# aponte411/minGPT-distributed

Measured on AMD Instinct MI355X. Metric: tokens/sec (whole node), GPT-2 124M seq1024 bf16, higher is better.
Workload: dtype bf16; 1 GPU; model=gpt2, global_batch=128, seq_len=1024, parallelism=dp1, micro_batch_per_gpu=128, hip_graph=False

## Files before the change

### csrc/bindings.cpp

```cpp
#include <torch/extension.h>
#include <ATen/hip/impl/HIPGuardImplMasqueradingAsCUDA.h>
#include <ATen/hip/impl/HIPStreamMasqueradingAsCUDA.h>

#include "comm.h"
#include "kernels.h"

namespace {

using mg::bf16_t;

hipStream_t cur_stream() { return c10::hip::getCurrentHIPStreamMasqueradingAsCUDA().stream(); }
using DevGuard = c10::hip::HIPGuardMasqueradingAsCUDA;

#define CHECK_DEV(t) TORCH_CHECK((t).is_cuda(), #t " must be a GPU tensor")
#define CHECK_CONTIG(t) TORCH_CHECK((t).is_contiguous(), #t " must be contiguous")
#define CHECK_BF16(t) \
  CHECK_DEV(t);       \
  TORCH_CHECK((t).scalar_type() == at::kBFloat16, #t " must be bf16")
#define CHECK_F32(t) \
  CHECK_DEV(t);      \
  TORCH_CHECK((t).scalar_type() == at::kFloat, #t " must be fp32")
#define CHECK_I64(t) \
  CHECK_DEV(t);      \
  TORCH_CHECK((t).scalar_type() == at::kLong, #t " must be int64")
// ... 858 lines not shown
  m.def("xent_scale_", &xent_scale_);
  m.def("set_graph_state", &set_graph_state, py::arg("seed_ofs") = py::none(), py::arg("opt_hp") = py::none());
  m.def("grad_sumsq", &grad_sumsq);
  m.def("grad_sumsq_chunks", &grad_sumsq_chunks);
  m.def("adamw_step", &adamw_step, py::arg("chunk_start"), py::arg("chunk_len"), py::arg("chunk_wd"),
        py::arg("moment_start"), py::arg("master"), py::arg("param"), py::arg("grad"), py::arg("m"),
        py::arg("v"), py::arg("norm"), py::arg("lr"), py::arg("b1"), py::arg("b2"), py::arg("eps"),
        py::arg("step"), py::arg("grad_scale"), py::arg("clip"), py::arg("table_end"),
        py::arg("moment_end"), py::arg("zero_grad") = py::none());
  m.def("f32_to_bf16", &f32_to_bf16);
  m.def("comm_proxy", &comm_proxy);
  m.def("bias_act", &bias_act);
  m.def("bias_dropout_residual", &bias_dropout_residual);
  m.def("gelu_bwd", &gelu_bwd);
  m.def("dropout_bwd", &dropout_bwd);
  m.def("transpose", &transpose);
  m.def("bias_grad", &bias_grad);
  m.def("dropout_bias_grad", &dropout_bias_grad);
  m.def("gemm", &gemm, py::arg("a"), py::arg("b"), py::arg("c"), py::arg("layout"), py::arg("epi"),
        py::arg("bias"), py::arg("aux"), py::arg("resid"), py::arg("p"), py::arg("seed"), py::arg("M"),
        py::arg("N"), py::arg("dbias") = py::none());
  m.def("gemm_set_variant", &mg::gemm_set_variant);
  m.def("gemm_get_variant", &mg::gemm_get_variant);
  m.def("gemm_pick", &mg::gemm_pick, py::arg("M"), py::arg("N"), py::arg("K"), py::arg("layout"));
  m.def("attention_set_bwd_mode", &mg::attention_set_bwd_mode);
  m.def("attention_set_bwd64", &mg::attention_set_bwd64);
#ifdef MG_BWD64_STAMPS
  m.def("attention_bwd64_stamps", []() {
    auto t = at::empty({64 * 4 * 8 * 8 + 64 * 4 * 16}, at::kLong);
    mg::attention_bwd64_stamps(reinterpret_cast<unsigned long long*>(t.data_ptr<int64_t>()));
    return t;
  });
#endif
  m.def("attention_fwd", &attention_fwd);
  m.def("attention_bwd", &attention_bwd, py::arg("qkv"), py::arg("out"), py::arg("dout"), py::arg("lse"),
        py::arg("mask"), py::arg("B"), py::arg("T"), py::arg("H"), py::arg("p"), py::arg("seed"),
        py::arg("dbias") = py::none());
  m.def("gemv", &gemv, py::arg("x"), py::arg("W"), py::arg("epi"), py::arg("bias") = py::none(),
        py::arg("resid") = py::none(), py::arg("ldy") = 0, py::arg("lnw") = py::none(),
        py::arg("lnb") = py::none(), py::arg("eps") = 1e-5, py::arg("am_part") = py::none(),
        py::arg("am_pos") = py::none());
  m.def("gemv_argmax_groups", [](int64_t N, int64_t B) { return (int64_t)mg::gemv_grid((int)N, (int)B); },
        py::arg("N"), py::arg("B"));
  m.def("gemv_supported", &mg::gemv_supported);
  m.def("attention_decode", &attention_decode, py::arg("qkv_new"), py::arg("cache"), py::arg("H"),
        py::arg("pos"), py::arg("pos_dev") = py::none(), py::arg("part") = py::none(),
// ... 22 lines not shown
```

### csrc/include/kernels.h

```cpp
#pragma once
#include <hip/hip_runtime.h>
#include <stddef.h>
#include <stdint.h>

namespace mg {
typedef uint16_t bf16_t;

void layernorm_fwd(const bf16_t* x, const bf16_t* w, const bf16_t* b, bf16_t* y, float* mean,
                   float* rstd, int M, int D, float eps, hipStream_t stream);
void layernorm_bwd(const bf16_t* dy, const bf16_t* x, const bf16_t* w, const float* mean,
                   const float* rstd, const bf16_t* dres, bf16_t* dx, float* dw, float* db,
                   float* workspace, int M, int D, hipStream_t stream, bf16_t* dz = nullptr,
                   float* dzb = nullptr, float p = 0.f, uint64_t seed = 0);
size_t layernorm_bwd_workspace(int M, int D, bool drop);

void embedding_fwd(const int64_t* idx, const bf16_t* wte, const bf16_t* wpe, bf16_t* out, int M,
                   int T, int D, int V, float p, uint64_t seed, hipStream_t stream,
                   const int* pos_dev = nullptr,
                   const unsigned long long* am_part = nullptr,
                   int am_groups = 0,
                   int64_t* tok = nullptr,
                   int64_t* seq = nullptr,
                   long seq_ld = 0,
                   int pos_stride = 0,
// ... 56 lines not shown
void beam_merge(int B, int W, int V, const int* cand_tok, const float* cand_c, float* score, int* fin, int* len,
                int64_t* tok, int* parent, int* hist_parent, int* hist_tok, float* hist_score, long hist_ld, int* pos,
                const int* ctl, hipStream_t stream);
void beam_reorder(bf16_t* kv, int L, long layer_stride, int B, int W, int Tmax, int D, const int* parent,
                  const int* pos, int* ctl, hipStream_t stream);

void bias_act_fwd(const bf16_t* x, const bf16_t* b, bf16_t* pre, bf16_t* y, long M, int N, int act,
                  hipStream_t stream);
void bias_dropout_residual(const bf16_t* x, const bf16_t* b, const bf16_t* r, bf16_t* y, long M,
                           int N, float p, uint64_t seed, hipStream_t stream);
void gelu_bwd(const bf16_t* dy, const bf16_t* pre, bf16_t* dx, long n, hipStream_t stream);
void dropout_bwd(const bf16_t* dy, bf16_t* dx, long M, int N, float p, uint64_t seed, hipStream_t stream);
void transpose(const bf16_t* src, bf16_t* dst, int R, int C, int ldd, hipStream_t stream);
void bias_grad(const bf16_t* dy, float* db, long M, int N, hipStream_t stream, long ld = 0);
void dropout_bias_grad(const bf16_t* dy, bf16_t* dx, float* db, long M, int N, float p, uint64_t seed,
                       hipStream_t stream);

void gemm(int layout, int epi, const bf16_t* A, const bf16_t* B, void* C, long lda, long ldb,
          long ldc, int M, int N, int K, int a_ext, int b_ext, int ka, int kb, const bf16_t* bias,
          bf16_t* aux, const bf16_t* resid, float p, uint64_t seed, hipStream_t stream,
          size_t a_bytes, size_t b_bytes,
          float* dbias = nullptr);
void gemm_set_variant(int v);
void gemm_set_debug_buffer(unsigned long long* p);
int gemm_get_variant();
int gemm_pick(int M, int N, int K, int layout);

size_t attention_dropout_mask_words(int B, int T, int H);
int attention_dropout_threshold(float p);
float attention_dropout_scale(int thr);
void attention_fwd(const bf16_t* qkv, bf16_t* out, float* lse, uint32_t* dmask, int B, int T, int H,
                   int hd, float p, uint64_t seed, hipStream_t stream);
size_t attention_bwd_workspace_floats(int B, int T, int H, int hd);
void attention_set_bwd_mode(int mode);
void attention_set_bwd64(int on);
#ifdef MG_BWD64_STAMPS
void attention_bwd64_stamps(unsigned long long* host);
#endif
void attention_bwd(const bf16_t* qkv, const bf16_t* out, const bf16_t* dout, const float* lse,
                   const uint32_t* dmask, float* delta, float* dq, bf16_t* dqkv, int B, int T, int H,
                   int hd, float p, uint64_t seed, hipStream_t stream, float* dbias = nullptr);

size_t attention_decode_part_floats(int B, int H, int hd);
void attention_decode(const bf16_t* qkv_new, bf16_t* cache, bf16_t* out, int B, int H, int hd,
                      long Tmax, int pos, hipStream_t stream, float* part, unsigned* counters,
                      const int* pos_dev = nullptr, int pos_stride = 0);
// ... 3 lines not shown
```

### csrc/kernels/gemm.hip

```cpp
#include "common.h"
#include "kernels.h"
#include <type_traits>


using namespace mg;

namespace {

typedef __bf16 bf16x8 __attribute__((ext_vector_type(8)));
typedef __attribute__((address_space(3))) s16x4 lds_s16x4;
typedef __attribute__((address_space(3))) void lds_void;

constexpr int BK = 64;
#ifndef MG_GROUP_M
#define MG_GROUP_M 8
#endif
constexpr int GROUP_M = MG_GROUP_M;
constexpr uint32_t kOOB = 0xFFFFFFF0u;

template <int BM_, int BN_, int NWM_, int NWN_, int STAGES_ = 2>
struct Cfg {
  static constexpr int BM = BM_, BN = BN_, NWM = NWM_, NWN = NWN_, STAGES = STAGES_;
  static constexpr int NW = NWM * NWN, NT = NW * 64;
  static constexpr int WTM = BM / NWM, WTN = BN / NWN;
// ... 58 lines not shown
    ptr = reinterpret_cast<const char*>(p);
    total = tot;
    ld = ld_;
    kbeg = kbeg_;
    step = KC ? BK * 2 : (uint32_t)(BK * ld * 2);
    klim = min(kvalid, kend) - kbeg;
    tail_t = klim / BK;
    swid = __builtin_amdgcn_readfirstlane(wid);
#pragma unroll
    for (int i = 0; i < PER; ++i) {
      const int j = wid * PER + i;
      if constexpr (KC) {
        const int row = 8 * j + (lane >> 3), ch = (lane & 7) ^ (row & 7);
        voff[i] = (uint32_t)(((long)row * ld + ch * 8) * 2);
      } else {
        const int half = j >> 4, jj = j & 15;
        const int row = 4 * jj + (lane >> 4), ch = (lane & 15) ^ swz_mn(row);
        const int gc = r0 + half * 128 + ch * 8;
        voff[i] = gc < ext ? (uint32_t)(((long)row * ld + gc) * 2) : kOOB;
      }
    }
    retarget(r0);
  }
  MG_DEVICE void retarget(int r0) {
    const uint64_t o = KC ? (uint64_t)((long)r0 * ld + kbeg) * 2 : (uint64_t)kbeg * ld * 2;
    base = ptr + o;
    const uint64_t rest = total > o ? total - o : 0u;
    bytes = rest < 0xFFFFFF00u ? (uint32_t)rest : 0xFFFFFF00u;
  }
  MG_DEVICE __amdgpu_buffer_rsrc_t rsrc(int t) const { return tile_rsrc(base, bytes, step, t); }
  MG_DEVICE void piece(char* lds, __amdgpu_buffer_rsrc_t rs, int t, int i, bool check = true) const {
    const int j = swid * PER + i;
    uint32_t off = voff[i];
    if (check && t >= tail_t) {
      const int lane = threadIdx.x & 63;
      const int kpos = KC ? ((lane & 7) ^ ((lane >> 3) & 7)) * 8 : 4 * (j & 15) + (lane >> 4);
      off = kpos < klim - t * BK ? off : kOOB;
    }
    char* dst = KC ? lds + j * 1024 : lds + (j >> 4) * HS + (j & 15) * 1024;
    __builtin_amdgcn_raw_ptr_buffer_load_lds(rs, (lds_void*)dst, 16, off, 0, 0, 0);
  }
  MG_DEVICE void stage(char* lds, int t) const {
    const __amdgpu_buffer_rsrc_t rs = tile_rsrc(base, bytes, step, t);
#pragma unroll
    for (int i = 0; i < PER; ++i) piece(lds, rs, t, i);
  }
};

MG_DEVICE uint32_t lds_addr(const void* p) {
  return (uint32_t)(uintptr_t)(const __attribute__((address_space(3))) void*)p;
}
// ... 43 lines not shown
MG_DEVICE uint4 load8(const bf16_t* p, int valid) {
  if (valid >= 8) return *reinterpret_cast<const uint4*>(p);
  uint16_t t[8];
#pragma unroll
  for (int e = 0; e < 8; ++e) t[e] = e < valid ? p[e] : (uint16_t)0;
  return make_uint4(t[0] | (uint32_t)t[1] << 16, t[2] | (uint32_t)t[3] << 16, t[4] | (uint32_t)t[5] << 16,
                    t[6] | (uint32_t)t[7] << 16);
}

MG_DEVICE void store8(bf16_t* p, uint4 v, int valid) {
  if (valid >= 8) {
    *reinterpret_cast<uint4*>(p) = v;
    return;
  }
  const uint32_t w[4] = {v.x, v.y, v.z, v.w};
#pragma unroll
  for (int e = 0; e < 8; ++e)
    if (e < valid) p[e] = (uint16_t)(w[e >> 1] >> (16 * (e & 1)));
}

template <class CF>
constexpr bool staged_dbias() { return 64 % (CF::WTN / 8) == 0; }

template <int EPI, int S, int CHF, int PR, int IT, bool NT>
MG_DEVICE void staged_copy_out(const GemmArgs& args, const char* st, int mr, int nw, int lane) {
  constexpr int RPI = 64 / PR, G = 8;
  static_assert(IT % G == 0, "pieces per lane must be a multiple of the read group");
  const int r0 = lane / PR, p = lane % PR;
  const char* lrow = st + r0 * S + p * 16;
  const long off0 = (long)(mr + r0) * args.ldc + nw + p * 8;
  bf16_t* gc = reinterpret_cast<bf16_t*>(args.C) + off0;
  bf16_t* ga = EPI == 2 ? args.aux + off0 : nullptr;
  const long rs = (long)RPI * args.ldc;
  typedef unsigned v4u __attribute__((ext_vector_type(4)));
#pragma unroll
  for (int g0 = 0; g0 < IT; g0 += G) {
    uint4 y[G], z[EPI == 2 ? G : 1];
#pragma unroll
    for (int u = 0; u < G; ++u) {
      y[u] = *reinterpret_cast<const uint4*>(lrow + (g0 + u) * RPI * S);
      if constexpr (EPI == 2) z[u] = *reinterpret_cast<const uint4*>(lrow + CHF * 16 * S + (g0 + u) * RPI * S);
    }
#pragma unroll
    for (int u = 0; u < G; ++u) {
      const long o = (long)(g0 + u) * rs;
      if constexpr (NT) {
        __builtin_nontemporal_store(v4u{y[u].x, y[u].y, y[u].z, y[u].w}, reinterpret_cast<v4u*>(gc + o));
        if constexpr (EPI == 2)
          __builtin_nontemporal_store(v4u{z[u].x, z[u].y, z[u].z, z[u].w}, reinterpret_cast<v4u*>(ga + o));
// ... 26 lines not shown
    for (int u = 0; u < G; ++u) {
      float v[8] = {a[u].x, a[u].y, a[u].z, a[u].w, b[u].x, b[u].y, b[u].z, b[u].w};
      if constexpr (EPI != 7) {
        const uint4 sv = sd[g0 + u];
        const uint32_t w[4] = {sv.x, sv.y, sv.z, sv.w};
#pragma unroll
        for (int k = 0; k < 8; ++k) {
          const float s = bf2f((w[k >> 1] >> (16 * (k & 1))) & 0xffffu);
          v[k] = EPI == 3 ? v[k] + s : v[k] * s;
        }
      }
      if constexpr ((EPI == 4 || EPI == 7) && staged_dbias<CF>()) {
#pragma unroll
        for (int k = 0; k < 8; ++k) cs[k] += v[k];
      }
      const uint4 y = make_uint4(pack2(v[0], v[1]), pack2(v[2], v[3]), pack2(v[4], v[5]), pack2(v[6], v[7]));
      bf16_t* dst = gc + (long)(g0 + u) * rs;
      if constexpr (NT) __builtin_nontemporal_store(v4u{y.x, y.y, y.z, y.w}, reinterpret_cast<v4u*>(dst));
      else *reinterpret_cast<uint4*>(dst) = y;
    }
  }
}

template <class CF, int EPI, bool F32, int S, int CHF, int PR, int IT, bool CHECK>
MG_DEVICE void staged_rows(const GemmArgs& args, const char* st, const uint4 (&sd)[F32 ? IT : 1], int mr,
                           int nw, int nlim, int lane, float (&cs)[8]) {
  if constexpr (!F32 && !CHECK && 64 % PR == 0 && IT % 8 == 0) {
    if (args.nt_out) staged_copy_out<EPI, S, CHF, PR, IT, true>(args, st, mr, nw, lane);
    else staged_copy_out<EPI, S, CHF, PR, IT, false>(args, st, mr, nw, lane);
    return;
  }
  if constexpr (EPI == 4 && !CHECK && 64 % PR == 0 && IT % 2 == 0) {
    if (args.nt_out) staged_side_out<CF, EPI, S, PR, IT, true>(args, st, sd, mr, nw, lane, cs);
    else staged_side_out<CF, EPI, S, PR, IT, false>(args, st, sd, mr, nw, lane, cs);
    return;
  }
#pragma unroll
  for (int it = 0; it < IT; ++it) {
    const int e = it * 64 + lane, r = e / PR, p = e % PR;
    const int m = mr + r, n = nw + p * 8;
    const char* row = st + r * S;
    uint4 y;
    if constexpr (F32) {
      const float4 a = *reinterpret_cast<const float4*>(row + p * 32);
      const float4 b = *reinterpret_cast<const float4*>(row + p * 32 + 16);
      float v[8] = {a.x, a.y, a.z, a.w, b.x, b.y, b.z, b.w};
      const uint32_t w[4] = {sd[it].x, sd[it].y, sd[it].z, sd[it].w};
#pragma unroll
      for (int k = 0; k < 8; ++k) {
        const float s = bf2f((w[k >> 1] >> (16 * (k & 1))) & 0xffffu);
        if constexpr (EPI != 7) v[k] = EPI == 3 ? v[k] + s : v[k] * s;
      }
// ... 14 lines not shown
    const long off = (long)m * args.ldc + n;
    if constexpr (!CHECK) {
      if (args.nt_out) {
        typedef unsigned v4u __attribute__((ext_vector_type(4)));
        __builtin_nontemporal_store(v4u{y.x, y.y, y.z, y.w},
                                    reinterpret_cast<v4u*>(reinterpret_cast<bf16_t*>(args.C) + off));
        if constexpr (EPI == 2) {
          const uint4 g = *reinterpret_cast<const uint4*>(row + CHF * 16 * S + p * 16);
          __builtin_nontemporal_store(v4u{g.x, g.y, g.z, g.w}, reinterpret_cast<v4u*>(args.aux + off));
        }
      } else {
        *reinterpret_cast<uint4*>(reinterpret_cast<bf16_t*>(args.C) + off) = y;
        if constexpr (EPI == 2)
          *reinterpret_cast<uint4*>(args.aux + off) = *reinterpret_cast<const uint4*>(row + CHF * 16 * S + p * 16);
      }
    } else if (m < args.M && n < nlim) {
      store8(reinterpret_cast<bf16_t*>(args.C) + off, y, nlim - n);
      if constexpr (EPI == 2)
        store8(args.aux + off, *reinterpret_cast<const uint4*>(row + CHF * 16 * S + p * 16), nlim - n);
    }
  }
}

template <class CF, int EPI, int LDSW>
MG_DEVICE void epilogue_staged(const GemmArgs& args, f32x4 (&acc)[CF::FM][CF::FN], int m0, int n0,
                               int wm, int wn, int wid, int lane, char* smem,
                               unsigned long long* est = nullptr) {
  constexpr bool F32 = EPI == 4;
  constexpr int PL = EPI == 2 ? 2 : 1;
  constexpr int S = CF::WTN * (F32 ? 4 : 2) + 16;
  constexpr int CHF = stage_chf(CF::FM, 16 * S * PL, LDSW);
  constexpr int PR = CF::WTN / 8;
  constexpr int IT = CHF * 16 * PR / 64;
  static_assert(CHF * 16 * S * PL <= LDSW, "epilogue staging exceeds the wave's LDS share");
  static_assert((CHF * 16 * PR) % 64 == 0, "pieces must fill whole waves");
  char* st = smem + wid * LDSW;
  const int nlim = EPI == 0 ? (int)args.ldc : args.N;
  const int nw = n0 + wn * CF::WTN;
  const int nb = nw + (lane >> 4) * 4;
  const int mw = m0 + wm * CF::WTM;
  uint2 bs[CF::FN];
#pragma unroll
  for (int j = 0; j < CF::FN; ++j) {
    bs[j] = make_uint2(0u, 0u);
    if constexpr (EPI == 1 || EPI == 2 || EPI == 3 || EPI == 6)
      if (args.bias && nb + j * 16 < nlim) bs[j] = *reinterpret_cast<const uint2*>(args.bias + nb + j * 16);
  }
  const bool full = nw + CF::WTN <= nlim && mw + CF::WTM <= args.M;
  const bf16_t* __restrict__ side = args.aux;
  constexpr bool ROLL = EPI == 3 || EPI == 7;
  uint2 rsd[ROLL ? 2 : 1][ROLL ? CF::FN : 1];
  bf16_t* const frag_aux = (EPI == 6 || EPI == 7)
      ? args.aux + ((long)(m0 / 256) * args.tiles_n + n0 / 256) * 65536 + (long)wid * CF::FM * CF::FN * 256 + lane * 8
      : nullptr;
  auto resid_load = [&](int i, uint2 (&dst)[ROLL ? CF::FN : 1]) __attribute__((always_inline)) {
    if constexpr (EPI == 7) {
#pragma unroll
      for (int j = 0; j < CF::FN; j += 2) {
        const uint4 t = *reinterpret_cast<const uint4*>(frag_aux + (i * CF::FN + j) * 256);
        dst[j] = make_uint2(t.x, t.y);
        dst[j + 1] = make_uint2(t.z, t.w);
      }
    }
    if constexpr (EPI == 3) {
      const int m = mw + i * 16 + (lane & 15);
#pragma unroll
      for (int j = 0; j < CF::FN; ++j) {
        const int n = nb + j * 16;
        const bf16_t* p = args.resid + (long)m * args.ldc + n;
        if (full) {
          dst[j] = *reinterpret_cast<const uint2*>(p);
        } else if (m < args.M && n < nlim) {
          const uint4 t = load8(p, min(4, nlim - n));
          dst[j] = make_uint2(t.x, t.y);
        } else {
          dst[j] = make_uint2(0u, 0u);
        }
      }
    }
  };
  const uint32_t dkey = EPI == 3 ? rowdrop_key(eff_seed(args.seed, args.sofs)) : 0u;
  float cs[8] = {0.f, 0.f, 0.f, 0.f, 0.f, 0.f, 0.f, 0.f};
  float csf[EPI == 7 ? 4 * CF::FN : 1];
#pragma unroll
  for (int k = 0; k < (EPI == 7 ? 4 * CF::FN : 1); ++k) csf[k] = 0.f;
  resid_load(0, rsd[0]);
#pragma unroll
  for (int c = 0; c < CF::FM / CHF; ++c) {
    uint4 sd[F32 ? IT : 1];
    if constexpr (EPI == 4) {
#pragma unroll
      for (int it = 0; it < IT; ++it) {
        const int e = it * 64 + lane, r = e / PR, n = nw + (e % PR) * 8;
        const int m = mw + c * CHF * 16 + r;
        const bf16_t* p = side + (long)m * args.ldc + n;
        if (full) sd[it] = *reinterpret_cast<const uint4*>(p);
        else sd[it] = m < args.M && n < nlim ? load8(p, nlim - n) : make_uint4(0u, 0u, 0u, 0u);
      }
    }
#pragma unroll
    for (int ii = 0; ii < CHF; ++ii) {
      const int i = c * CHF + ii;
      const int m = mw + i * 16 + (lane & 15);
      char* row = st + (ii * 16 + (lane & 15)) * S;
      if constexpr (ROLL) {
        if (i + 1 < CF::FM) resid_load(i + 1, rsd[(i + 1) & 1]);
      }
      uint32_t gq[4];
// ... 34 lines not shown
          v[0] = y0.x; v[1] = y0.y; v[2] = y1.x; v[3] = y1.y;
          *reinterpret_cast<uint2*>(row + CHF * 16 * S + col * 2) =
              make_uint2(pack2(g0.x, g0.y), pack2(g1.x, g1.y));
        }
        if constexpr (EPI == 3) {
          if (args.thr) rowdrop4(v, dkey, m, n, args.N, args.thr, args.scale);
          const uint2 rv = rsd[i & 1][j];
          v[0] += bf2f(rv.x & 0xffffu); v[1] += bf2f(rv.x >> 16);
          v[2] += bf2f(rv.y & 0xffffu); v[3] += bf2f(rv.y >> 16);
        }
        if constexpr (F32)
          *reinterpret_cast<float4*>(row + col * 4) = make_float4(v[0], v[1], v[2], v[3]);
        else
          *reinterpret_cast<uint2*>(row + col * 2) = make_uint2(pack2(v[0], v[1]), pack2(v[2], v[3]));
      }
    }
#ifdef MG_GEMM_EPI_STAMPS
    if (est && c == 0) est[0] = __builtin_amdgcn_s_memtime();
#endif
    asm volatile("s_waitcnt lgkmcnt(0)" ::: "memory");
#ifdef MG_GEMM_EPI_STAMPS
    if (est && c == 0) est[1] = __builtin_amdgcn_s_memtime();
#endif
    if (full) staged_rows<CF, EPI, F32, S, CHF, PR, IT, false>(args, st, sd, mw + c * CHF * 16, nw, nlim, lane, cs);
    else staged_rows<CF, EPI, F32, S, CHF, PR, IT, true>(args, st, sd, mw + c * CHF * 16, nw, nlim, lane, cs);
    asm volatile("" ::: "memory");
#ifdef MG_GEMM_EPI_STAMPS
    if (est) est[2] = __builtin_amdgcn_s_memtime();
#endif
  }
  if constexpr (EPI == 7) {
    if (args.dbias) {
      constexpr int NV = 4 * CF::FN;
      static_assert(NV == 32, "fragment-layout fold: 8 fragments per wave-tile row");
#pragma unroll
      for (int M = 8; M >= 1; M >>= 1) {
        const bool hi = lane & M;
        const int C = NV * M / 8;
#pragma unroll
        for (int i2 = 0; i2 < C / 2; ++i2) {
          const float send = hi ? csf[i2] : csf[i2 + C / 2];
          const float keep = hi ? csf[i2 + C / 2] : csf[i2];
          csf[i2] = keep + __shfl_xor(send, M, 64);
        }
      }
      float* red = reinterpret_cast<float*>(smem);
      __syncthreads();
#pragma unroll
      for (int t = 0; t < 2; ++t) {
        const int idx = 2 * (lane & 15) + t, j = idx / 4, e = idx % 4;
        red[wm * CF::BN + wn * CF::WTN + 16 * j + 4 * (lane >> 4) + e] = csf[t];
      }
      __syncthreads();
// ... 8 lines not shown
  if constexpr (EPI == 4 && staged_dbias<CF>()) {
    if (args.dbias) {
#pragma unroll
      for (int k = 0; k < 8; ++k)
#pragma unroll
        for (int o = PR; o < 64; o <<= 1) cs[k] += __shfl_xor(cs[k], o, 64);
      float* red = reinterpret_cast<float*>(smem);
      __syncthreads();
      if (lane < PR) {
#pragma unroll
        for (int k = 0; k < 8; ++k) red[wm * CF::BN + wn * CF::WTN + lane * 8 + k] = cs[k];
      }
      __syncthreads();
      for (int c = threadIdx.x; c < CF::BN; c += CF::NT) {
        float t = 0.f;
#pragma unroll
        for (int r = 0; r < CF::NWM; ++r) t += red[r * CF::BN + c];
        if (n0 + c < args.N) atomicAdd(args.dbias + n0 + c, t);
      }
    }
  }
}

template <class CF, int EPI, bool OUTF32, int LDSW>
MG_DEVICE void epilogue(const GemmArgs& args, f32x4 (&acc)[CF::FM][CF::FN], int m0, int n0, int wm,
                        int wn, int wid, int lane, char* smem, unsigned long long* est = nullptr) {
  if constexpr (!OUTF32) {
    if ((EPI != 4 && EPI != 7) || !args.dbias || staged_dbias<CF>()) {
      epilogue_staged<CF, EPI, LDSW>(args, acc, m0, n0, wm, wn, wid, lane, smem, est);
      return;
    }
  }
  if constexpr (OUTF32) {
    if (args.splits > 1) {
      constexpr int RS = CF::WTN + 4;
      float* ct = reinterpret_cast<float*>(smem) + wid * 32 * RS;
      float* C = reinterpret_cast<float*>(args.C);
#pragma unroll
      for (int pass = 0; pass < CF::FM / 2; ++pass) {
#pragma unroll
        for (int ii = 0; ii < 2; ++ii)
#pragma unroll
          for (int j = 0; j < CF::FN; ++j)
            *reinterpret_cast<f32x4*>(ct + (ii * 16 + (lane & 15)) * RS + j * 16 + (lane >> 4) * 4) =
                acc[pass * 2 + ii][j];
        __syncthreads();
        for (int c = lane; c < CF::WTN; c += 64) {
          const int n = n0 + wn * CF::WTN + c;
          for (int r = 0; r < 32; ++r) {
            const int m = m0 + wm * CF::WTM + pass * 32 + r;
            if (m < args.M && n < args.N) atomicAdd(C + (long)m * args.ldc + n, ct[r * RS + c]);
          }
// ... 224 lines not shown
  static constexpr int FN = BN / 32;
  static constexpr int A_SLOT = 32768;
  static constexpr int B_SLOT = BN * 128;
  static constexpr int B_RING = 2 * A_SLOT;
  static constexpr int SMEM = 2 * A_SLOT + 3 * B_SLOT;
  static constexpr int NR = 8 + FN;
  static constexpr int PA = 8, PB = FN;
};

template <int NQ, int NR>
MG_DEVICE constexpr int w4_piece_at(int q) {
  for (int r = 0; r < NR; ++r)
    if (r * NQ / NR == q) return r;
  return -1;
}

MG_DEVICE int w4_tile(int s, int nk, bool tail_first) { return tail_first ? (s == 0 ? nk - 1 : s - 1) : s; }

MG_DEVICE void mfma_acc_last(f32x4& acc, const bf16x8& a, const bf16x8& b) {
  asm volatile("v_mfma_f32_16x16x32_bf16 %0, %1, %2, %0\n\ts_nop 7\n\ts_nop 7" : "+a"(acc) : "v"(a), "v"(b) : "memory");
}


template <int BN, bool AK, bool BKC, int EPI, bool OUTF32>
__global__ __launch_bounds__(256, 1) void gemm_w4_kernel(const GemmArgs args) {
  static_assert(BN == 256 || BKC, "W4 with BN != 256 needs a k-contiguous B operand");
  using CF = Cfg<256, BN, 2, 2>;
  using WK = W4<BN>;
  constexpr int FN = WK::FN, NR = WK::NR, NQ = 8 * FN;
  extern __shared__ __attribute__((aligned(16))) char smem[];
  const int lane = threadIdx.x & 63, wid = threadIdx.x >> 6;
  const int wm = wid >> 1, wn = wid & 1;

  const int nblk = args.tiles_m * args.tiles_n * args.splits;
  const int orig = blockIdx.x;
  const int xcd = orig & 7, q8 = nblk >> 3, r8 = nblk & 7;
  const int wgs = (xcd < r8 ? xcd * (q8 + 1) : r8 * (q8 + 1) + (xcd - r8) * q8) + (orig >> 3);
  const int ntiles = args.tiles_m * args.tiles_n;
  const int split = wgs / ntiles;
  const int wg = wgs % ntiles;
  const int group = GROUP_M * args.tiles_n;
  const int first_m = (wg / group) * GROUP_M;
  const int gm = min(args.tiles_m - first_m, GROUP_M);
  const int m0 = (first_m + (wg % group) % gm) * 256;
  const int n0 = ((wg % group) / gm) * BN;

#ifdef MG_GEMM_STAMPS
  unsigned long long st[10];
#define W4_STAMP(k) st[k] = __builtin_amdgcn_s_memtime()
#define W4_KSTAMP(k) if (kt == MG_GEMM_STAMPS) st[k] = __builtin_amdgcn_s_memtime()
#else
#define W4_STAMP(k)
#define W4_KSTAMP(k)
#endif
  W4_STAMP(6);
  f32x4 acc[8][FN];
#pragma unroll
  for (int i = 0; i < 8; ++i)
#pragma unroll
    for (int j = 0; j < FN; ++j) acc[i][j] = f32x4{0.f, 0.f, 0.f, 0.f};

  const int kbeg = split * args.kchunk;
  const int nk = (min(args.K, kbeg + args.kchunk) - kbeg + BK - 1) / BK;
  constexpr int AS = AK ? WK::A_SLOT : 16384, AHS = 2 * 16384;
  constexpr int BS = BKC ? WK::B_SLOT : 16384, BHS = 3 * 16384;
  Stager<AK, 256, 4, AHS> sta;
  Stager<BKC, BN, 4, BHS> stb;
  sta.init(args.A, args.a_bytes, args.lda, m0, args.a_ext, kbeg, args.ka, kbeg + args.kchunk, wid, lane);
  stb.init(args.B, args.b_bytes, args.ldb, n0, args.b_ext, kbeg, args.kb, kbeg + args.kchunk, wid, lane);
  const bool tail_first = (sta.klim % BK) != 0;
  char* const sB = smem + WK::B_RING;
  sta.stage(smem, w4_tile(0, nk, tail_first));
  stb.stage(sB, w4_tile(0, nk, tail_first));
  if (nk > 1) {
    sta.stage(smem + AS, w4_tile(1, nk, tail_first));
    stb.stage(sB + BS, w4_tile(1, nk, tail_first));
    asm volatile("s_waitcnt vmcnt(%0)" ::"n"(WK::PA + WK::PB) : "memory");
  } else {
    asm volatile("s_waitcnt vmcnt(0)" ::: "memory");
  }
  __builtin_amdgcn_s_barrier();
  asm volatile("" ::: "memory");

  bf16x8 fa0[8], fb0[FN], fa1[8], fb1[FN];
#pragma unroll
  for (int j = 0; j < FN; ++j) fb0[j] = frag_k<BKC, 0, BHS>(sB, wn * FN + j, lane);
#pragma unroll
  for (int i = 0; i < 8; ++i) fa0[i] = frag_k<AK, 0, AHS>(smem, wm * 8 + i, lane);
  lds_ready(fa0);
  lds_ready(fb0, false);
  W4_STAMP(7);

  auto ktile = [&](int kt, auto sa_c, auto sb_c) __attribute__((always_inline)) {
    constexpr int SA = decltype(sa_c)::value, SB = decltype(sb_c)::value;
    constexpr int OA = SA * AS, OA1 = (SA ^ 1) * AS;
    constexpr int OB = SB * BS, OB1 = ((SB + 1) % 3) * BS, OB2 = ((SB + 2) % 3) * BS;
    W4_KSTAMP(0);
    const int t2 = kt + 2;
    const int tt = w4_tile(t2 < nk ? t2 : 1, nk, tail_first);
    {
      const __amdgpu_buffer_rsrc_t rb = stb.rsrc(tt);
#pragma unroll
      for (int q = 0; q < NQ; ++q) {
        const int i = q / FN, j = q % FN;
        mfma_acc(acc[i][j], fb0[j], fa0[i]);
        if ((q & 1) == 0 && q < 2 * NR) {
          const int r = q >> 1;
          if (r < FN) fb1[r] = frag_k<BKC, 1, BHS, OB>(sB, wn * FN + r, lane);
          else fa1[r - FN] = frag_k<AK, 1, AHS, OA>(smem, wm * 8 + r - FN, lane);
        }
        if (w4_piece_at<NQ, WK::PB>(q) >= 0) stb.piece(sB + OB2, rb, tt, w4_piece_at<NQ, WK::PB>(q), false);
      }
    }
    W4_KSTAMP(1);
    asm volatile("s_waitcnt vmcnt(%0) lgkmcnt(0)" ::"n"(WK::PB) : "memory");
    lds_ready(fa1, false);
    lds_ready(fb1, false);
    W4_KSTAMP(2);
    __builtin_amdgcn_s_barrier();
    asm volatile("" ::: "memory");
    W4_KSTAMP(3);
    {
      const __amdgpu_buffer_rsrc_t ra = sta.rsrc(tt);
#pragma unroll
      for (int q = 0; q < NQ; ++q) {
        const int i = q / FN, j = q % FN;
        if (q == NQ - 1) mfma_acc_last(acc[i][j], fb1[j], fa1[i]);
        else mfma_acc(acc[i][j], fb1[j], fa1[i]);
        if (w4_piece_at<NQ, WK::PA>(q) >= 0) sta.piece(smem + OA, ra, tt, w4_piece_at<NQ, WK::PA>(q), false);
        if (q < 2 * NR && (q & 1) == 1) {
          const int r = q >> 1;
          if (r < FN) fb0[r] = frag_k<BKC, 0, BHS, OB1>(sB, wn * FN + r, lane);
          else fa0[r - FN] = frag_k<AK, 0, AHS, OA1>(smem, wm * 8 + r - FN, lane);
        }
      }
    }
    W4_KSTAMP(4);
    lds_ready(fa0);
    lds_ready(fb0, false);
    W4_KSTAMP(5);
  };
  using I0 = std::integral_constant<int, 0>;
  using I1 = std::integral_constant<int, 1>;
  using I2 = std::integral_constant<int, 2>;

  int kt = 0;
  for (; kt + 6 <= nk; kt += 6) {
    ktile(kt, I0{}, I0{});
    ktile(kt + 1, I1{}, I1{});
    ktile(kt + 2, I0{}, I2{});
    ktile(kt + 3, I1{}, I0{});
    ktile(kt + 4, I0{}, I1{});
    ktile(kt + 5, I1{}, I2{});
  }
  if (kt < nk) ktile(kt, I0{}, I0{});
  if (kt + 1 < nk) ktile(kt + 1, I1{}, I1{});
  if (kt + 2 < nk) ktile(kt + 2, I0{}, I2{});
  if (kt + 3 < nk) ktile(kt + 3, I1{}, I0{});
  if (kt + 4 < nk) ktile(kt + 4, I0{}, I1{});
  W4_STAMP(8);
  asm volatile("s_waitcnt vmcnt(0) lgkmcnt(0)" ::: "memory");
  __syncthreads();
#ifdef MG_GEMM_EPI_STAMPS
  epilogue<CF, EPI, OUTF32, WK::SMEM / 4>(args, acc, m0, n0, wm, wn, wid, lane, smem, st);
#else
  epilogue<CF, EPI, OUTF32, WK::SMEM / 4>(args, acc, m0, n0, wm, wn, wid, lane, smem);
#endif
#ifdef MG_GEMM_STAMPS
  asm volatile("s_waitcnt vmcnt(0)" ::: "memory");
  W4_STAMP(9);
  if (args.dbg && lane == 0)
    for (int k = 0; k < 10; ++k) args.dbg[((long)blockIdx.x * 8 + wid) * 24 + k] = st[k];
#endif
#undef W4_STAMP
#undef W4_KSTAMP
}

template <int BN, bool AK, bool BKC, int EPI, bool OUTF32>
void launch_w4(GemmArgs a, hipStream_t stream) {
  if constexpr (BN != 256 && !BKC) {
    launch_w4<256, AK, BKC, EPI, OUTF32>(a, stream);
  } else {
    a.tiles_m = cdiv(a.M, 256);
    a.tiles_n = cdiv(a.N, BN);
    a.splits = 1;
    a.kchunk = cdiv(a.K, BK) * BK;
    if (OUTF32) set_split(a, 256, 6);
    const int tiles = a.tiles_m * a.tiles_n * a.splits;
    const int grid = tiles;
    static bool attr_set = false;
    if (!attr_set) {
      hipFuncSetAttribute((const void*)gemm_w4_kernel<BN, AK, BKC, EPI, OUTF32>,
                          hipFuncAttributeMaxDynamicSharedMemorySize, W4<BN>::SMEM);
      attr_set = true;
    }
    gemm_w4_kernel<BN, AK, BKC, EPI, OUTF32><<<grid, 256, W4<BN>::SMEM, stream>>>(a);
  }
}

template <class CF, bool AK, bool BKC, int EPI, bool OUTF32>
void launch(GemmArgs a, hipStream_t stream) {
  a.tiles_m = cdiv(a.M, CF::BM);
  a.tiles_n = cdiv(a.N, CF::BN);
  a.splits = 1;
  a.kchunk = cdiv(a.K, BK) * BK;
  if (OUTF32) set_split(a, 256 * (CF::SMEM <= 80 * 1024 ? 2 : 1), 2 + CF::BM * CF::BN / 16384);
  const int grid = a.tiles_m * a.tiles_n * a.splits;
  static bool attr_set = false;
  if (!attr_set) {
    hipFuncSetAttribute((const void*)gemm_kernel<CF, AK, BKC, EPI, OUTF32>,
                        hipFuncAttributeMaxDynamicSharedMemorySize, CF::SMEM);
// ... 20 lines not shown
  return c1 * 65 < c4 * 100 ? 1 : 5;
}

template <bool AK, bool BKC, int EPI, bool OUTF32>
void dispatch(const GemmArgs& a, hipStream_t stream) {
  const int layout = OUTF32 ? 2 : (BKC ? 0 : 1);
  switch (pick_config(a.M, a.N, a.K, layout)) {
    case 5: launch_w4<256, AK, BKC, EPI, OUTF32>(a, stream); break;
    case 6: launch_w4<192, AK, BKC, EPI, OUTF32>(a, stream); break;
    default: launch<T128, AK, BKC, EPI, OUTF32>(a, stream); break;
  }
}

}

namespace mg {

int gemm_pick(int M, int N, int K, int layout) { return pick_config(M, N, K, layout); }

void gemm_set_variant(int v) {
  if (v != 0 && v != 1 && v != 5 && v != 6) throw std::invalid_argument("gemm_set_variant: 0 (auto), 1 (T128), 5 (W4), 6 (W4 BN=192)");
  g_variant = v;
}
void gemm_set_debug_buffer(unsigned long long* p) { g_dbg = p; }
int gemm_get_variant() { return g_variant; }

void gemm(int layout, int epi, const bf16_t* A, const bf16_t* B, void* C, long lda, long ldb,
          long ldc, int M, int N, int K, int a_ext, int b_ext, int ka, int kb, const bf16_t* bias,
          bf16_t* aux, const bf16_t* resid, float p, uint64_t seed, hipStream_t stream,
          size_t a_bytes, size_t b_bytes, float* dbias) {
  GemmArgs a;
  a.dbias = dbias;
  a.a_bytes = a_bytes;
  a.b_bytes = b_bytes;
  a.A = A; a.B = B; a.C = C; a.lda = lda; a.ldb = ldb; a.ldc = ldc;
  a.M = M; a.N = N; a.K = K; a.a_ext = a_ext; a.b_ext = b_ext; a.ka = ka; a.kb = kb;
  a.bias = bias; a.aux = aux; a.resid = resid; a.seed = seed; a.sofs = graph_seed_ofs();
  a.thr = dropout_threshold16(p);
  a.scale = dropout_scale16(a.thr);
  a.tiles_m = a.tiles_n = a.splits = 1;
  a.kchunk = K;
  a.dbg = g_dbg;
  a.nt_out = 1;
  if (layout == 0) {
    if (epi == 0) dispatch<true, true, 0, false>(a, stream);
    else if (epi == 1) dispatch<true, true, 1, false>(a, stream);
// ... 15 lines not shown
```

Measured before the change: 1.127 million tokens/s.

## Add persistent chained W4 GEMM that prefetches the next tile during epilogue

Adds a persistent variant of the W4 GEMM kernel. A grid of one workgroup per CU walks several output tiles in turn, and the k-loop's prefetch of the last stages already loads the A/B tiles of the next output tile, so loads overlap the current tile's epilogue. The epilogue is restaged into a spare B slot and uses a smaller read group. By default this is enabled only when K/BK equals 12 and there are at least twice as many tiles as CUs, which targets GPT-2's K=768 GEMMs. In exchange it adds complexity and custom waitcnt and barrier logic that could hurt correctness, and the persistent grid loses some load balance.

After: 1.131 million tokens/s, median of 6. Within noise of the previous version (+0.3%).

```diff
diff --git a/csrc/bindings.cpp b/csrc/bindings.cpp
--- a/csrc/bindings.cpp
+++ b/csrc/bindings.cpp
@@ -904,6 +904,8 @@
         py::arg("N"), py::arg("dbias") = py::none());
   m.def("gemm_set_variant", &mg::gemm_set_variant);
   m.def("gemm_get_variant", &mg::gemm_get_variant);
+  m.def("gemm_set_chain", &mg::gemm_set_chain, py::arg("mode"), py::arg("max_workgroups") = 0);
+  m.def("gemm_chain_used", &mg::gemm_chain_used);
   m.def("gemm_pick", &mg::gemm_pick, py::arg("M"), py::arg("N"), py::arg("K"), py::arg("layout"));
   m.def("attention_set_bwd_mode", &mg::attention_set_bwd_mode);
   m.def("attention_set_bwd64", &mg::attention_set_bwd64);
diff --git a/csrc/include/kernels.h b/csrc/include/kernels.h
--- a/csrc/include/kernels.h
+++ b/csrc/include/kernels.h
@@ -102,6 +102,8 @@
           size_t a_bytes, size_t b_bytes,
           float* dbias = nullptr);
 void gemm_set_variant(int v);
+void gemm_set_chain(int mode, int max_workgroups);
+long gemm_chain_used();
 void gemm_set_debug_buffer(unsigned long long* p);
 int gemm_get_variant();
 int gemm_pick(int M, int N, int K, int layout);
diff --git a/csrc/kernels/gemm.hip b/csrc/kernels/gemm.hip
--- a/csrc/kernels/gemm.hip
+++ b/csrc/kernels/gemm.hip
@@ -104,11 +104,12 @@
     }
     retarget(r0);
   }
-  MG_DEVICE void retarget(int r0) {
+  MG_DEVICE void retarget(int r0) { origin(r0, base, bytes); }
+  MG_DEVICE void origin(int r0, const char*& b, uint32_t& n) const {
     const uint64_t o = KC ? (uint64_t)((long)r0 * ld + kbeg) * 2 : (uint64_t)kbeg * ld * 2;
-    base = ptr + o;
+    b = ptr + o;
     const uint64_t rest = total > o ? total - o : 0u;
-    bytes = rest < 0xFFFFFF00u ? (uint32_t)rest : 0xFFFFFF00u;
+    n = rest < 0xFFFFFF00u ? (uint32_t)rest : 0xFFFFFF00u;
   }
   MG_DEVICE __amdgpu_buffer_rsrc_t rsrc(int t) const { return tile_rsrc(base, bytes, step, t); }
   MG_DEVICE void piece(char* lds, __amdgpu_buffer_rsrc_t rs, int t, int i, bool check = true) const {
@@ -198,9 +199,9 @@
 template <class CF>
 constexpr bool staged_dbias() { return 64 % (CF::WTN / 8) == 0; }
 
-template <int EPI, int S, int CHF, int PR, int IT, bool NT>
+template <int EPI, int S, int CHF, int PR, int IT, bool NT, int G = 8>
 MG_DEVICE void staged_copy_out(const GemmArgs& args, const char* st, int mr, int nw, int lane) {
-  constexpr int RPI = 64 / PR, G = 8;
+  constexpr int RPI = 64 / PR;
   static_assert(IT % G == 0, "pieces per lane must be a multiple of the read group");
   const int r0 = lane / PR, p = lane % PR;
   const char* lrow = st + r0 * S + p * 16;
@@ -273,12 +274,17 @@
   }
 }
 
-template <class CF, int EPI, bool F32, int S, int CHF, int PR, int IT, bool CHECK>
+template <class CF, int EPI, bool F32, int S, int CHF, int PR, int IT, bool CHECK, bool CHAIN = false>
 MG_DEVICE void staged_rows(const GemmArgs& args, const char* st, const uint4 (&sd)[F32 ? IT : 1], int mr,
                            int nw, int nlim, int lane, float (&cs)[8]) {
   if constexpr (!F32 && !CHECK && 64 % PR == 0 && IT % 8 == 0) {
     if (args.nt_out) staged_copy_out<EPI, S, CHF, PR, IT, true>(args, st, mr, nw, lane);
     else staged_copy_out<EPI, S, CHF, PR, IT, false>(args, st, mr, nw, lane);
+    return;
+  }
+  if constexpr (CHAIN && !F32 && !CHECK && 64 % PR == 0 && IT == 4) {
+    if (args.nt_out) staged_copy_out<EPI, S, CHF, PR, IT, true, 4>(args, st, mr, nw, lane);
+    else staged_copy_out<EPI, S, CHF, PR, IT, false, 4>(args, st, mr, nw, lane);
     return;
   }
   if constexpr (EPI == 4 && !CHECK && 64 % PR == 0 && IT % 2 == 0) {
@@ -339,7 +345,7 @@
   }
 }
 
-template <class CF, int EPI, int LDSW>
+template <class CF, int EPI, int LDSW, bool CHAIN = false>
 MG_DEVICE void epilogue_staged(const GemmArgs& args, f32x4 (&acc)[CF::FM][CF::FN], int m0, int n0,
                                int wm, int wn, int wid, int lane, char* smem,
                                unsigned long long* est = nullptr) {
@@ -363,13 +369,21 @@
     if constexpr (EPI == 1 || EPI == 2 || EPI == 3 || EPI == 6)
       if (args.bias && nb + j * 16 < nlim) bs[j] = *reinterpret_cast<const uint2*>(args.bias + nb + j * 16);
   }
-  const bool full = nw + CF::WTN <= nlim && mw + CF::WTM <= args.M;
+  const bool full_rt = nw + CF::WTN <= nlim && mw + CF::WTM <= args.M;
   const bf16_t* __restrict__ side = args.aux;
   constexpr bool ROLL = EPI == 3 || EPI == 7;
   uint2 rsd[ROLL ? 2 : 1][ROLL ? CF::FN : 1];
+  const uint32_t dkey = EPI == 3 ? rowdrop_key(eff_seed(args.seed, args.sofs)) : 0u;
+  float cs[8] = {0.f, 0.f, 0.f, 0.f, 0.f, 0.f, 0.f, 0.f};
+  float csf[EPI == 7 ? 4 * CF::FN : 1];
+#pragma unroll
+  for (int k = 0; k < (EPI == 7 ? 4 * CF::FN : 1); ++k) csf[k] = 0.f;
   bf16_t* const frag_aux = (EPI == 6 || EPI == 7)
       ? args.aux + ((long)(m0 / 256) * args.tiles_n + n0 / 256) * 65536 + (long)wid * CF::FM * CF::FN * 256 + lane * 8
       : nullptr;
+  auto passes = [&](auto mode_c) __attribute__((always_inline)) {
+  constexpr int MODE = decltype(mode_c)::value;
+  const bool full = MODE == 0 ? full_rt : MODE == 1;
   auto resid_load = [&](int i, uint2 (&dst)[ROLL ? CF::FN : 1]) __attribute__((always_inline)) {
     if constexpr (EPI == 7) {
 #pragma unroll
@@ -396,11 +410,6 @@
       }
     }
   };
-  const uint32_t dkey = EPI == 3 ? rowdrop_key(eff_seed(args.seed, args.sofs)) : 0u;
-  float cs[8] = {0.f, 0.f, 0.f, 0.f, 0.f, 0.f, 0.f, 0.f};
-  float csf[EPI == 7 ? 4 * CF::FN : 1];
-#pragma unroll
-  for (int k = 0; k < (EPI == 7 ? 4 * CF::FN : 1); ++k) csf[k] = 0.f;
   resid_load(0, rsd[0]);
 #pragma unroll
   for (int c = 0; c < CF::FM / CHF; ++c) {
@@ -481,13 +490,20 @@
 #ifdef MG_GEMM_EPI_STAMPS
     if (est && c == 0) est[1] = __builtin_amdgcn_s_memtime();
 #endif
-    if (full) staged_rows<CF, EPI, F32, S, CHF, PR, IT, false>(args, st, sd, mw + c * CHF * 16, nw, nlim, lane, cs);
-    else staged_rows<CF, EPI, F32, S, CHF, PR, IT, true>(args, st, sd, mw + c * CHF * 16, nw, nlim, lane, cs);
+    if (full) staged_rows<CF, EPI, F32, S, CHF, PR, IT, false, CHAIN>(args, st, sd, mw + c * CHF * 16, nw, nlim, lane, cs);
+    else staged_rows<CF, EPI, F32, S, CHF, PR, IT, true, CHAIN>(args, st, sd, mw + c * CHF * 16, nw, nlim, lane, cs);
     asm volatile("" ::: "memory");
 #ifdef MG_GEMM_EPI_STAMPS
     if (est) est[2] = __builtin_amdgcn_s_memtime();
 #endif
   }
+  };
+  if constexpr (CHAIN) {
+    if (full_rt) passes(std::integral_constant<int, 1>{});
+    else passes(std::integral_constant<int, 2>{});
+  } else {
+    passes(std::integral_constant<int, 0>{});
+  }
   if constexpr (EPI == 7) {
     if (args.dbias) {
       constexpr int NV = 4 * CF::FN;
@@ -542,12 +558,12 @@
   }
 }
 
-template <class CF, int EPI, bool OUTF32, int LDSW>
+template <class CF, int EPI, bool OUTF32, int LDSW, bool CHAIN = false>
 MG_DEVICE void epilogue(const GemmArgs& args, f32x4 (&acc)[CF::FM][CF::FN], int m0, int n0, int wm,
                         int wn, int wid, int lane, char* smem, unsigned long long* est = nullptr) {
   if constexpr (!OUTF32) {
     if ((EPI != 4 && EPI != 7) || !args.dbias || staged_dbias<CF>()) {
-      epilogue_staged<CF, EPI, LDSW>(args, acc, m0, n0, wm, wn, wid, lane, smem, est);
+      epilogue_staged<CF, EPI, LDSW, CHAIN>(args, acc, m0, n0, wm, wn, wid, lane, smem, est);
       return;
     }
   }
@@ -818,9 +834,11 @@
 }
 
 
-template <int BN, bool AK, bool BKC, int EPI, bool OUTF32>
+template <int BN, bool AK, bool BKC, int EPI, bool OUTF32, bool CHAIN = false>
 __global__ __launch_bounds__(256, 1) void gemm_w4_kernel(const GemmArgs args) {
   static_assert(BN == 256 || BKC, "W4 with BN != 256 needs a k-contiguous B operand");
+  static_assert(!CHAIN || (BN == 256 && AK && BKC && !OUTF32 && (EPI == 0 || EPI == 1 || EPI == 3 || EPI == 6)),
+                "chained W4: BN = 256, k-contiguous operands, bf16 output, per-wave epilogues");
   using CF = Cfg<256, BN, 2, 2>;
   using WK = W4<BN>;
   constexpr int FN = WK::FN, NR = WK::NR, NQ = 8 * FN;
@@ -829,17 +847,24 @@
   const int wm = wid >> 1, wn = wid & 1;
 
   const int nblk = args.tiles_m * args.tiles_n * args.splits;
-  const int orig = blockIdx.x;
-  const int xcd = orig & 7, q8 = nblk >> 3, r8 = nblk & 7;
-  const int wgs = (xcd < r8 ? xcd * (q8 + 1) : r8 * (q8 + 1) + (xcd - r8) * q8) + (orig >> 3);
   const int ntiles = args.tiles_m * args.tiles_n;
-  const int split = wgs / ntiles;
-  const int wg = wgs % ntiles;
   const int group = GROUP_M * args.tiles_n;
-  const int first_m = (wg / group) * GROUP_M;
-  const int gm = min(args.tiles_m - first_m, GROUP_M);
-  const int m0 = (first_m + (wg % group) % gm) * 256;
-  const int n0 = ((wg % group) / gm) * BN;
+  auto tile_of = [&](int orig, int& sp, int& tm0, int& tn0) __attribute__((always_inline)) {
+    const int xcd = orig & 7, q8 = nblk >> 3, r8 = nblk & 7;
+    const int wgs = (xcd < r8 ? xcd * (q8 + 1) : r8 * (q8 + 1) + (xcd - r8) * q8) + (orig >> 3);
+    sp = wgs / ntiles;
+    const int wg = wgs % ntiles;
+    const int first_m = (wg / group) * GROUP_M;
+    const int gm = min(args.tiles_m - first_m, GROUP_M);
+    tm0 = (first_m + (wg % group) % gm) * 256;
+    tn0 = ((wg % group) / gm) * BN;
+  };
+  int vb = blockIdx.x;
+  if constexpr (CHAIN) {
+    if (vb >= nblk) return;
+  }
+  int split, m0, n0;
+  tile_of(vb, split, m0, n0);
 
 #ifdef MG_GEMM_STAMPS
   unsigned long long st[10];
@@ -851,10 +876,15 @@
 #endif
   W4_STAMP(6);
   f32x4 acc[8][FN];
-#pragma unroll
-  for (int i = 0; i < 8; ++i)
-#pragma unroll
-    for (int j = 0; j < FN; ++j) acc[i][j] = f32x4{0.f, 0.f, 0.f, 0.f};
+  auto acc_clear = [&]() __attribute__((always_inline)) {
+#pragma unroll
+    for (int i = 0; i < 8; ++i)
+#pragma unroll
+      for (int j = 0; j < FN; ++j) {
+        acc[i][j] = f32x4{0.f, 0.f, 0.f, 0.f};
+      }
+  };
+  acc_clear();
 
   const int kbeg = split * args.kchunk;
   const int nk = (min(args.K, kbeg + args.kchunk) - kbeg + BK - 1) / BK;
@@ -878,11 +908,29 @@
   __builtin_amdgcn_s_barrier();
   asm volatile("" ::: "memory");
 
+  int vbn = 0, m1 = 0, n1 = 0;
+  bool more = false, chained_in = false;
+  auto plan_next = [&]() __attribute__((always_inline)) {
+    vbn = vb + (int)gridDim.x;
+    more = vbn < nblk;
+    if (more) {
+      int sp1;
+      tile_of(vbn, sp1, m1, n1);
+    }
+  };
+  if constexpr (CHAIN) plan_next();
+
   bf16x8 fa0[8], fb0[FN], fa1[8], fb1[FN];
-#pragma unroll
-  for (int j = 0; j < FN; ++j) fb0[j] = frag_k<BKC, 0, BHS>(sB, wn * FN + j, lane);
-#pragma unroll
-  for (int i = 0; i < 8; ++i) fa0[i] = frag_k<AK, 0, AHS>(smem, wm * 8 + i, lane);
+  for (;;) {
+  {
+    int l0 = lane;
+    if constexpr (CHAIN) asm volatile("v_mbcnt_lo_u32_b32 %0, -1, 0\n\tv_mbcnt_hi_u32_b32 %0, -1, %0" : "=v"(l0));
+    const int w0 = CHAIN ? sta.swid : wid;
+#pragma unroll
+    for (int j = 0; j < FN; ++j) fb0[j] = frag_k<BKC, 0, BHS>(sB, (w0 & 1) * FN + j, l0);
+#pragma unroll
+    for (int i = 0; i < 8; ++i) fa0[i] = frag_k<AK, 0, AHS>(smem, (w0 >> 1) * 8 + i, l0);
+  }
   lds_ready(fa0);
   lds_ready(fb0, false);
   W4_STAMP(7);
@@ -893,9 +941,18 @@
     constexpr int OB = SB * BS, OB1 = ((SB + 1) % 3) * BS, OB2 = ((SB + 2) % 3) * BS;
     W4_KSTAMP(0);
     const int t2 = kt + 2;
-    const int tt = w4_tile(t2 < nk ? t2 : 1, nk, tail_first);
+    const bool nx = CHAIN && more && t2 >= nk;
+    const int tt = nx ? t2 - nk : w4_tile(t2 < nk ? t2 : 1, nk, tail_first);
     {
-      const __amdgpu_buffer_rsrc_t rb = stb.rsrc(tt);
+      __amdgpu_buffer_rsrc_t rb;
+      if constexpr (CHAIN) {
+        const char* ob;
+        uint32_t on;
+        stb.origin(nx ? n1 : n0, ob, on);
+        rb = tile_rsrc(ob, on, stb.step, tt);
+      } else {
+        rb = stb.rsrc(tt);
+      }
 #pragma unroll
       for (int q = 0; q < NQ; ++q) {
         const int i = q / FN, j = q % FN;
@@ -909,7 +966,8 @@
       }
     }
     W4_KSTAMP(1);
-    asm volatile("s_waitcnt vmcnt(%0) lgkmcnt(0)" ::"n"(WK::PB) : "memory");
+    if (CHAIN && SA == 0 && SB == 0 && kt == 0 && chained_in) asm volatile("s_waitcnt lgkmcnt(0)" ::: "memory");
+    else asm volatile("s_waitcnt vmcnt(%0) lgkmcnt(0)" ::"n"(WK::PB) : "memory");
     lds_ready(fa1, false);
     lds_ready(fb1, false);
     W4_KSTAMP(2);
@@ -917,7 +975,15 @@
     asm volatile("" ::: "memory");
     W4_KSTAMP(3);
     {
-      const __amdgpu_buffer_rsrc_t ra = sta.rsrc(tt);
+      __amdgpu_buffer_rsrc_t ra;
+      if constexpr (CHAIN) {
+        const char* oa;
+        uint32_t on;
+        sta.origin(nx ? m1 : m0, oa, on);
+        ra = tile_rsrc(oa, on, sta.step, tt);
+      } else {
+        ra = sta.rsrc(tt);
+      }
 #pragma unroll
       for (int q = 0; q < NQ; ++q) {
         const int i = q / FN, j = q % FN;
@@ -949,6 +1015,28 @@
     ktile(kt + 4, I0{}, I1{});
     ktile(kt + 5, I1{}, I2{});
   }
+  if constexpr (CHAIN) {
+    asm volatile("s_waitcnt lgkmcnt(0)" ::: "memory");
+    __builtin_amdgcn_s_barrier();
+    asm volatile("" ::: "memory");
+    int ln;
+    asm volatile("v_mbcnt_lo_u32_b32 %0, -1, 0\n\tv_mbcnt_hi_u32_b32 %0, -1, %0" : "=v"(ln));
+    const int sw = sta.swid;
+    epilogue<CF, EPI, OUTF32, WK::B_SLOT / 4, true>(args, acc, m0, n0, sw >> 1, sw & 1, sw, ln, sB + 2 * BS);
+    const int nlim = EPI == 0 ? (int)args.ldc : args.N;
+    const bool full = n0 + (sw & 1) * 128 + 128 <= nlim && m0 + (sw >> 1) * 128 + 128 <= args.M;
+    if (full) asm volatile("s_waitcnt vmcnt(%0)" ::"n"(EPI == 0 || EPI == 1 ? 32 : 63) : "memory");
+    else asm volatile("s_waitcnt vmcnt(0)" ::: "memory");
+    if (!more) break;
+    __builtin_amdgcn_s_barrier();
+    asm volatile("" ::: "memory");
+    vb = vbn;
+    m0 = m1;
+    n0 = n1;
+    chained_in = true;
+    plan_next();
+    acc_clear();
+  } else {
   if (kt < nk) ktile(kt, I0{}, I0{});
   if (kt + 1 < nk) ktile(kt + 1, I1{}, I1{});
   if (kt + 2 < nk) ktile(kt + 2, I0{}, I2{});
@@ -962,6 +1050,9 @@
 #else
   epilogue<CF, EPI, OUTF32, WK::SMEM / 4>(args, acc, m0, n0, wm, wn, wid, lane, smem);
 #endif
+  break;
+  }
+  }
 #ifdef MG_GEMM_STAMPS
   asm volatile("s_waitcnt vmcnt(0)" ::: "memory");
   W4_STAMP(9);
@@ -970,6 +1061,42 @@
 #endif
 #undef W4_STAMP
 #undef W4_KSTAMP
+}
+
+static int g_chain_mode = 0, g_chain_maxwg = 0;
+static long g_chain_used = 0;
+
+static int device_cus() {
+  static int ncu[64] = {0};
+  int dev = 0;
+  (void)hipGetDevice(&dev);
+  if (dev < 0 || dev >= 64) dev = 0;
+  if (!ncu[dev]) {
+    int n = 0;
+    (void)hipDeviceGetAttribute(&n, hipDeviceAttributeMultiprocessorCount, dev);
+    ncu[dev] = n > 0 ? n : 256;
+  }
+  return ncu[dev];
+}
+
+template <int EPI>
+static bool chain_rule(int nk, long tiles, int ncu) {
+  (void)tiles; (void)ncu;
+  return nk == 12;
+}
+
+template <int BN, bool AK, bool BKC, int EPI, bool OUTF32>
+static int chain_grid(const GemmArgs& a, long tiles) {
+  if constexpr (BN == 256 && AK && BKC && !OUTF32 && (EPI == 0 || EPI == 1 || EPI == 3 || EPI == 6)) {
+    if (g_chain_mode == 2 || a.splits != 1 || a.K % BK != 0) return 0;
+    const int nk = a.K / BK;
+    if (nk < 6 || nk % 6 != 0) return 0;
+    const int ncu = device_cus();
+    if (g_chain_maxwg > 0) return g_chain_mode == 1 ? std::min(g_chain_maxwg, ncu) : 0;
+    if (tiles < 2L * ncu) return 0;
+    return (g_chain_mode == 1 || chain_rule<EPI>(nk, tiles, ncu)) ? ncu : 0;
+  }
+  return 0;
 }
 
 template <int BN, bool AK, bool BKC, int EPI, bool OUTF32>
@@ -983,6 +1110,19 @@
     a.kchunk = cdiv(a.K, BK) * BK;
     if (OUTF32) set_split(a, 256, 6);
     const int tiles = a.tiles_m * a.tiles_n * a.splits;
+    if constexpr (BN == 256 && AK && BKC && !OUTF32 && (EPI == 0 || EPI == 1 || EPI == 3 || EPI == 6)) {
+      if (const int cg = chain_grid<BN, AK, BKC, EPI, OUTF32>(a, tiles)) {
+        static bool attr_c = false;
+        if (!attr_c) {
+          hipFuncSetAttribute((const void*)gemm_w4_kernel<BN, AK, BKC, EPI, OUTF32, true>,
+                              hipFuncAttributeMaxDynamicSharedMemorySize, W4<BN>::SMEM);
+          attr_c = true;
+        }
+        ++g_chain_used;
+        gemm_w4_kernel<BN, AK, BKC, EPI, OUTF32, true><<<cg, 256, W4<BN>::SMEM, stream>>>(a);
+        return;
+      }
+    }
     const int grid = tiles;
     static bool attr_set = false;
     if (!attr_set) {
@@ -1049,6 +1189,13 @@
   if (v != 0 && v != 1 && v != 5 && v != 6) throw std::invalid_argument("gemm_set_variant: 0 (auto), 1 (T128), 5 (W4), 6 (W4 BN=192)");
   g_variant = v;
 }
+void gemm_set_chain(int mode, int max_workgroups) {
+  if (mode < 0 || mode > 2 || max_workgroups < 0)
+    throw std::invalid_argument("gemm_set_chain: mode 0 (rule), 1 (on where supported), 2 (off); max_workgroups >= 0");
+  g_chain_mode = mode;
+  g_chain_maxwg = max_workgroups;
+}
+long gemm_chain_used() { return g_chain_used; }
 void gemm_set_debug_buffer(unsigned long long* p) { g_dbg = p; }
 int gemm_get_variant() { return g_variant; }
 
```
